# NVIDIA/tensorrt-laboratory

Hardware: NVIDIA H100
Metric: ResNet-50 fp16 b=8 inferences/sec (higher is better)
Workload: dtype f16

## Files before the change

### __graft_entry__.py

```python
from __future__ import annotations

import os
import re
import shutil
import subprocess
import sysconfig
import sys

ROOT = os.path.dirname(os.path.abspath(__file__))
PKG = os.path.join(ROOT, "tensorrt_laboratory_b200")
CSRC = os.path.join(PKG, "csrc")
LIB = os.path.join(PKG, "libb200infer.so")

NVCC_FLAGS = [
    "-gencode", "arch=compute_90a,code=sm_90a", "-lineinfo", "-O3", "-std=c++17",
    "-Xcompiler", "-fPIC,-Wall,-Wno-unused-function", "-cudart", "static",
]


def _nvcc() -> str:
    for cand in (os.environ.get("NVCC"), shutil.which("nvcc"), "/usr/local/cuda/bin/nvcc"):
        if cand and os.path.exists(cand):
            return cand
    raise RuntimeError("nvcc not found")
# ... 20 lines not shown

def _all_deps():
    deps = []
    for root, _, files in os.walk(CSRC):
        deps += [os.path.join(root, f) for f in files if f.endswith((".cu", ".cc", ".h", ".cuh", ".hpp"))]
    deps.append(os.path.join(ROOT, "include", "b200infer.h"))
    inc = os.path.join(ROOT, "include")
    for root, _, files in os.walk(inc):
        deps += [os.path.join(root, f) for f in files]
    return deps


_CONV_KERNEL = re.compile(r"conv|net_f16_tcgen05|attention_f16_wgmma|embed_ln|layernorm_h8|pooler")


def _ptxas_violations(log: str):
    bad = [line.strip() for line in log.splitlines() if "(C7520)" in line]
    func = None
    for line in log.splitlines():
        m = re.search(r"Function properties for (\S+)", line)
        if m:
            func = m.group(1)
            continue
        m = re.search(r"(\d+) bytes spill stores, (\d+) bytes spill loads", line)
        if m and func and _CONV_KERNEL.search(func) and (int(m.group(1)) or int(m.group(2))):
            bad.append(f"{func}: {line.strip()}")
    return bad


def _compile_object(cmd, obj: str, verbose: bool) -> None:
    r = subprocess.run(cmd + ["-Xptxas", "-v"], capture_output=True, text=True)
    log = r.stdout + r.stderr
    shown = [line for line in log.splitlines() if verbose or not (line.startswith("ptxas info") or "bytes stack frame" in line)]
    if shown:
        sys.stderr.write("\n".join(shown) + "\n")
    if r.returncode:
        raise subprocess.CalledProcessError(r.returncode, cmd)
    bad = _ptxas_violations(log)
    if bad:
        os.remove(obj)
        raise RuntimeError(f"{os.path.basename(obj)}: ptxas reports serialised wgmma or spilling convolution / transformer kernels:\n  " +
                           "\n  ".join(bad))


def build(force: bool = False, verbose: bool = False) -> None:
    nvcc = _nvcc()
    objdir = os.path.join(ROOT, "build", "obj")
    os.makedirs(objdir, exist_ok=True)
    deps = _all_deps()
    objs = []
    for src in _sources():
        obj = os.path.join(objdir, os.path.relpath(src, CSRC).replace(os.sep, "_") + ".o")
        objs.append(obj)
        if force or _stale(obj, deps):
            cmd = [nvcc] + NVCC_FLAGS + ["-I", os.path.join(ROOT, "include"), "-I", CSRC]
            if src.endswith(".cc"):
# ... 52 lines not shown
```

### tensorrt_laboratory_b200/csrc/engine.cu

```cuda
#include <cuda.h>
#include <cuda_runtime.h>
#include <stdarg.h>
#include <stdio.h>
#include <stdlib.h>
#include <string.h>

#include <algorithm>
#include <map>
#include <memory>
#include <mutex>
#include <string>
#include <vector>

#include "../../include/b200infer.h"
#include "kernels.h"
#include "plan_format.h"

#include "b2_internal.h"

namespace b2i {
thread_local std::string g_err;
int fail(int code, const char* fmt, ...) {
    char buf[1024];
    va_list ap;
// ... 695 lines not shown
        if (cout_phys % bn || (group_span && group_span % bn)) continue;
        if (honor_forced && c->force_bn && bn != c->force_bn) continue;
        const int tiles = m_tiles * (cout_phys / bn);
        for (int splits = 1; splits <= 8; ++splits) {
            if (honor_forced && c->force_splits && !group_span ? splits != c->force_splits : splits != 1) continue;
            if (splits > 1 && (kb != 64 || kblocks / splits < 4 || tiles * splits > 160 || tiles > kMaxSplitTiles ||
                               size_t(tiles) * splits * 128 * bn * 4 > kSplitWorkspaceBytes))
                continue;
            const int kpc = (kblocks + splits - 1) / splits;
            if (splits > 1 && (splits - 1) * kpc >= kblocks) continue;
            for (int st : stgs) {
                if (!b2k::conv_config_exists(bn, kb, st)) continue;
                if (b2k::conv_smem_bytes(bn, st, residual) > kSmemLimit) continue;
                if (honor_forced && c->force_stages && st != c->force_stages) continue;
                if (!(honor_forced && c->force_stages) && !stage_depth_useful(bn, kb, st, kpc)) continue;
                const double smem = b2k::conv_smem_bytes(bn, st, residual);
                int per_sm = int(double(kSmemLimit) / smem);
                per_sm = std::min(per_sm, bn <= 64 ? 2 : 1);
                per_sm = std::max(1, std::min(per_sm, 8));
                const int ctas = tiles * splits;
                const int waves = (ctas + g_sms * per_sm - 1) / (g_sms * per_sm);
                const int sharing = std::max(1, std::min(per_sm, (ctas + g_sms - 1) / g_sms));
                const double stage_bytes = 16384.0 + bn * 128.0;
                const double t_kb = std::max(stage_bytes / (70000.0 / sharing), 1.0 / st);
                double t_epi = 0.6 + bn / 64.0 * 0.4 + (residual ? 0.4 : 0.0);
                if (splits > 1) t_epi += 1.0 + 0.3 * splits;
                const double t_cta = 2.0 + kpc * t_kb + t_epi;
                double total = waves * t_cta;
                const double traffic = double(ctas) * kpc * stage_bytes;
                total = std::max(total, traffic / 5.0e6 + 2.0);
                if (total < best.est_us) best = ConvConfig{bn, st, splits, total};
            }
        }
    }
// ... 290 lines not shown
        const uint64_t pix = uint64_t(r.cin_phys), rowb = uint64_t(ti.w) * pix, imgb = uint64_t(ti.h) * rowb;
        rc = make_map_im2col(&cl.mapA, tptr(r.in), int(r.cin_phys), int(ti.w), int(ti.h), batch, pix, rowb, imgb, op.kh(), op.kw(), op.sh(),
                             op.sw(), op.ph(), op.pw_lo(), op.pw_hi(), 128, 128, CU_TENSOR_MAP_SWIZZLE_128B, true);
    }
    if (rc) return rc;
    rc = make_map_2d(&cl.mapOut, tptr(r.out), r.cout_phys, uint64_t(M), 128, 128, CU_TENSOR_MAP_SWIZZLE_128B, true);
    if (rc) return rc;
    if (r.res >= 0) rc = make_map_2d(&cl.mapRes, tptr(r.res), r.cout_phys, uint64_t(M), 128, 128, CU_TENSOR_MAP_SWIZZLE_128B, true);
    else cl.mapRes = cl.mapOut;
    return rc;
}

struct TuneTimer {
    const int ns;
    const int iters = std::max(4, env_int("B2_TUNE_ITERS", 12));
    const int reps = std::max(1, env_int("B2_TUNE_REPS", 2));
    std::vector<cudaStream_t> ss;
    std::vector<cudaEvent_t> done;
    cudaEvent_t e0 = nullptr, e1 = nullptr;

    explicit TuneTimer(const b2_context* c) : ns(std::max(1, std::min(c->autotune, 8))), ss(size_t(ns), nullptr), done(size_t(ns), nullptr) {}
    ~TuneTimer() {
        for (auto s : ss)
            if (s) cudaStreamDestroy(s);
        for (auto d : done)
            if (d) cudaEventDestroy(d);
        if (e0) cudaEventDestroy(e0);
        if (e1) cudaEventDestroy(e1);
    }
    int init() {
        bool ok = cudaEventCreate(&e0) == cudaSuccess && cudaEventCreate(&e1) == cudaSuccess;
        for (int i = 0; i < ns && ok; ++i)
            ok = cudaStreamCreateWithFlags(&ss[size_t(i)], cudaStreamNonBlocking) == cudaSuccess &&
                 cudaEventCreateWithFlags(&done[size_t(i)], cudaEventDisableTiming) == cudaSuccess;
        if (ok) return B2_OK;
        cudaGetLastError();
        return fail(B2_ECUDA, "autotune: cannot create streams/events");
    }
    template <class F>
    cudaError_t time(F launch, float* ms) {
        int rc = 0;
        for (int i = 0; i < 2 && !rc; ++i)
            for (int k = 0; k < ns && !rc; ++k) rc = launch(k, ss[size_t(k)]);
        for (auto s : ss) cudaStreamSynchronize(s);
        *ms = 1e30f;
        cudaError_t se = cudaSuccess;
        for (int rep = 0; rep < reps && !rc && se == cudaSuccess; ++rep) {
            cudaEventRecord(e0, ss[0]);
            for (int k = 1; k < ns; ++k) cudaStreamWaitEvent(ss[size_t(k)], e0, 0);
            for (int i = 0; i < iters && !rc; ++i)
                for (int k = 0; k < ns && !rc; ++k) rc = launch(k, ss[size_t(k)]);
            for (int k = 1; k < ns; ++k) {
                cudaEventRecord(done[size_t(k)], ss[size_t(k)]);
                cudaStreamWaitEvent(ss[0], done[size_t(k)], 0);
            }
            cudaEventRecord(e1, ss[0]);
            se = cudaStreamSynchronize(ss[0]);
            float t = 0.f;
            if (se == cudaSuccess && cudaEventElapsedTime(&t, e0, e1) == cudaSuccess) *ms = std::min(*ms, t);
        }
        return rc ? cudaError_t(rc) : se;
    }
    double us_per_launch(double ms) const { return ms * 1e3 / (iters * ns); }
};

int autotune_conv(b2_context* c, const Op& op, int batch, int fixed_splits, ConvConfig* best_out) {
    const b2plan::OpRec& r = op.r;
    const Tensor& to = c->e->tensors[r.out];
    const int M = batch * int(to.h) * int(to.w);
    TuneTimer tt(c);
    int status = tt.init();
    if (status) return status;
    const int verbose = env_int("B2_TUNE_VERBOSE", 0);
    ConvConfig best = *best_out;
    double best_ms = 1e30;
// ... 1377 lines not shown
    const size_t bytes = size_t(run->ctas) * 64 * sizeof(long long);
    B2_CUDA(cudaMalloc(&d, bytes));
    cudaMemset(d, 0, bytes);
    cudaStream_t s = static_cast<cudaStream_t>(stream_);
    run->args.dbg = d;
    int rc = run_all(c, *plan, bindings, s);
    cudaError_t se = cudaStreamSynchronize(s);
    run->args.dbg = nullptr;
    if (!rc && se == cudaSuccess) cudaMemcpy(out, d, bytes, cudaMemcpyDeviceToHost);
    cudaFree(d);
    if (rc) return rc;
    if (se != cudaSuccess) return fail(B2_ECUDA, "debug launch failed: %s", cudaGetErrorString(se));
    return B2_OK;
}

const char* b2_context_launch_name(b2_context* c, int batch, int i) {
    static thread_local std::string s;
    const Launch* L = get_launch(c, batch, i);
    if (!L) return nullptr;
    static const char* kinds[] = {"input_cast", "conv_tcgen05", "conv_simt", "maxpool", "avgpool", "fc", "softmax", "output_cast", "net_tcgen05", "tail_pool_fc_softmax",
                                  "quantize", "conv_i8_tcgen05", "avgpool_i8", "output_cast_i8", "embed_ln", "layernorm", "attention_f16_wgmma",
                                  "pooler", "output_cast_rows"};
    s = std::string(kinds[L->kind]) + ":" + L->name;
    if (L->kind == L_CONV_TC)
        s += " bn=" + std::to_string(L->conv.bn) + " kb=" + std::to_string(L->conv.kb) +
             " st=" + std::to_string(L->conv.stages) + "x" + std::to_string(L->conv.sps) +
             (L->conv.ws_ctas ? " ws=" + std::to_string(L->conv.ws_ctas) : std::string()) +
             (L->conv.cn > 1 ? " cn=" + std::to_string(L->conv.cn) : std::string()) + (L->conv.halo ? " halo" : "") +
             (L->conv.args.a_mode == b2k::A_TILED ? " tiled" : " im2col") +
             " grid=" + std::to_string(L->conv.grid_n) + "x" + std::to_string(L->conv.grid_m) + "x" +
// ... 23 lines not shown
```

### tensorrt_laboratory_b200/csrc/kernels.cu

```cuda
#include "kernels.h"

#include <stdio.h>
#include <stdlib.h>
#include <string.h>

#include "ptx_sm90.cuh"
#include "wgmma_sm90.cuh"

namespace b2k {

template <int BN, int STAGES, int SPS = 1>
struct ConvCfg {
    static constexpr int A_SUBBLK = 128 * 64 * 2;
    static constexpr int B_SUBBLK = BN * 64 * 2;
    static constexpr int A_STAGE = SPS * A_SUBBLK;
    static constexpr int B_STAGE = SPS * B_SUBBLK;
    static constexpr int PIPE_BYTES = STAGES * (A_STAGE + B_STAGE);
    static constexpr int TILE_BYTES = 128 * BN * 2;
    static_assert(TILE_BYTES <= PIPE_BYTES, "the output staging tile reuses the pipeline buffers");
};

__host__ __device__ constexpr int conv_smem_layout_bytes(int bn, int stages, bool residual, int sps = 1) {
    return stages * sps * (128 * 64 * 2 + bn * 64 * 2) + (residual ? 128 * bn * 2 : 0) + 256 + bn * 4 + 1024;
}

constexpr int kConvThreads = 384;
constexpr int kConsumerWarps = 8;

struct FragPos {
    int row0, col0;
    __device__ FragPos(int consumer_warp, int lane)
        : row0(64 * (consumer_warp >> 2) + 16 * (consumer_warp & 3) + (lane >> 2)), col0(2 * (lane & 3)) {}
};

template <int BN, int KB, int STAGES, int SPS, int CN = 1, bool DBG = false, int AV = 0, bool GELU = false>
__global__ void __launch_bounds__(kConvThreads, BN <= 64 ? 2 : 1)
conv_f16_tcgen05(const __grid_constant__ CUtensorMap mapA, const __grid_constant__ CUtensorMap mapB,
                 const __grid_constant__ CUtensorMap mapOut, const __grid_constant__ CUtensorMap mapRes,
                 const ConvArgs p) {
    static_assert(SPS == 1 || KB == 64, "multi-sub-block stages exist for the 64-wide K path only");
    using Cfg = ConvCfg<BN, STAGES, SPS>;
    constexpr int TPS = 64 / KB;
    constexpr int A_SUB = 128 * KB * 2;
    constexpr int B_SUB = BN * KB * 2;
    constexpr int OW = BN >= 64 ? 64 : 32;
    constexpr int OROWB = OW * 2;
    constexpr int NBOX = BN / OW;

    extern __shared__ uint8_t smem_raw[];
    uint8_t* smem = smem_raw + ((1024u - (smem_u32(smem_raw) & 1023u)) & 1023u);
    const bool has_res = p.residual != nullptr;
// ... 42 lines not shown
    if (threadIdx.x == 0) {
        tma_prefetch_desc(&mapA);
        tma_prefetch_desc(&mapB);
        tma_prefetch_desc(&mapOut);
        if (has_res) tma_prefetch_desc(&mapRes);
        for (int s = 0; s < STAGES; ++s) {
            mbar_init(&full_bar[s], 1);
            mbar_init(&empty_bar[s], static_cast<uint32_t>(kConsumerWarps * cn));
        }
        mbar_init(res_bar, 1);
        fence_barrier_init();
        fence_proxy_async();
    }
    __syncthreads();
    if (cn > 1) cluster_sync_all();
    if (warp == 3) {
#pragma unroll
        for (int i = 0; i < BN / 32; ++i) s_bias[lane + 32 * i] = __ldg(p.bias + n0 + lane + 32 * i);
    }
    if (p.pdl_trigger == 0) pdl_launch_dependents();
    if (dbg && threadIdx.x == 0) dbg[1] = clock64();

    auto sub_tiles = [&](int kb) -> int {
        if (KB == 64) return 1;
        const int n = p.taps_phys - kb * TPS;
        return n > TPS ? TPS : n;
    };
    const bool skip_a = DBG && KB == 64 && (p.dbg_mode & 2), skip_b = DBG && KB == 64 && (p.dbg_mode & 4);
    auto stage_bytes = [&](int kb) -> uint32_t {
        if (KB == 64) {
            const int ns = subs_in_step((kb - kb_begin) / SPS);
// ... 13 lines not shown
                } else {
                    tma_load_2d(&mapB, &full_bar[s], b_dst + u * Cfg::B_SUBBLK, (kb + u) * 64, n0);
                }
            }
        } else {
            const int nt = sub_tiles(kb);
            for (int t = 0; t < nt; ++t) tma_load_2d(&mapB, &full_bar[s], b_dst + t * B_SUB, (kb * TPS + t) * KB, n0);
        }
    };
    auto load_residual = [&]() {
        mbar_expect_tx(res_bar, Cfg::TILE_BYTES);
#pragma unroll
        for (int b = 0; b < NBOX; ++b) tma_load_2d(&mapRes, res_bar, sRes + b * (128 * OROWB), n0 + b * OW, m0);
    };

    if (warp == 0) {
        {
            int img0 = 0, p0 = 0, q0 = 0;
            const int slice_rows = 128 / cn;
            int ms = m0 + static_cast<int>(crank) * slice_rows;
            const uint32_t slice_off = crank * static_cast<uint32_t>(slice_rows) * 128u;
            if (!a_tiled) {
                if (ms >= p.M) ms = 0;
                img0 = ms / p.HoWo;
                const int rem = ms - img0 * p.HoWo;
                p0 = rem / p.Wo;
                q0 = rem - p0 * p.Wo;
            }
            const int base_w = q0 * p.stride_w - p.pad_w;
            const int base_h = p0 * p.stride_h - p.pad_h;
            int cur_cb = 0, cur_r = 0, cur_sx = 0;
// ... 73 lines not shown
                    mbar_expect_tx(&full_bar[s], stage_bytes(kb_begin + i * SPS));
                    load_a(kb_begin + i * SPS, s);
                    if (!kSplitProducers) load_b(kb_begin + i * SPS, s);
                }
                __syncwarp();
                if (dbg) {
                    c3 = clock64();
                    tw += c1 - c0, tl += c3 - c1;
                }
            }
            if (dbg && lane == 0) dbg[11] = tw, dbg[12] = te, dbg[13] = tl;
        }
        __syncwarp();
    }

    const int cw = warp - 4;
    float acc[BN / 2];
    if (warp >= 4) {
        const uint32_t wg = static_cast<uint32_t>(cw >> 2);
        auto release_stage = [&](int st) {
            __syncwarp();
            if (lane == 0) {
                if (cn > 1) {
                    for (uint32_t r = 0; r < static_cast<uint32_t>(cn); ++r) mbar_arrive_cluster(&empty_bar[st], r);
                } else {
                    mbar_arrive(&empty_bar[st]);
                }
            }
        };
        long long mw = 0, mi = 0;
        for (int i = 0; i < nk; ++i) {
            const int s = i % STAGES;
            const uint32_t ph = (i / STAGES) & 1;
// ... 34 lines not shown
                wgmma_wait<0>();
                release_stage(0);
            } else {
                wgmma_wait<1>();
                if (i > 0) release_stage((i - 1) % STAGES);
            }
            if (dbg) mi += clock64() - m1c;
        }
        if constexpr (STAGES > 1) {
            wgmma_wait<0>();
            if (nk > 0) release_stage((nk - 1) % STAGES);
        }
        if (dbg && cw == 0 && lane == 0) dbg[4] = clock64(), dbg[14] = mw, dbg[15] = mi;
    }

    if (warp == 3 && KB == 64) {
        for (int i = 0; i < nk; ++i) {
            const int s = i % STAGES;
            if (i >= STAGES) mbar_wait(&empty_bar[s], ((i / STAGES) & 1) ^ 1);
            if (elect_one_sync()) load_b(kb_begin + i * SPS, s);
            __syncwarp();
        }
    }

    pdl_wait();
    __syncthreads();
    if (dbg && threadIdx.x == 128) dbg[5] = clock64();
    if (p.pdl_trigger == 1) pdl_launch_dependents();
    const FragPos fp(cw, lane);

    auto finish_pair = [&](int row, int col, float v0, float v1) {
        const int box = col / OW;
        const int chunk = (col % OW) / 8;
        const uint32_t so = static_cast<uint32_t>(box * (128 * OROWB)) + swz_off<OROWB>(row, chunk) + (col % 8) * 2;
        v0 += s_bias[col];
        v1 += s_bias[col + 1];
        if (has_res) {
            const float2 rf = __half22float2(*reinterpret_cast<const __half2*>(sRes + so));
            v0 += rf.x;
            v1 += rf.y;
        }
        if constexpr (GELU) {
            v0 = gelu_erf(v0);
            v1 = gelu_erf(v1);
        } else if (p.relu) {
            v0 = fmaxf(v0, 0.0f);
            v1 = fmaxf(v1, 0.0f);
        }
        *reinterpret_cast<__half2*>(sOut + so) = __floats2half2_rn(v0, v1);
    };

    bool do_store = true;
    if (!split) {
        if (warp >= 4) {
            if (has_res) mbar_wait(res_bar, 0);
#pragma unroll
            for (int j = 0; j < BN / 8; ++j)
#pragma unroll
                for (int h = 0; h < 2; ++h) finish_pair(fp.row0 + 8 * h, 8 * j + fp.col0, acc[4 * j + 2 * h], acc[4 * j + 2 * h + 1]);
        }
    } else {
        const int tile = blockIdx.y * gridDim.x + blockIdx.x;
        float* ws_tile = p.workspace + static_cast<size_t>(tile) * p.splits * (128 * BN);
        if (warp >= 4) {
            float* mine = ws_tile + static_cast<size_t>(blockIdx.z) * (128 * BN);
#pragma unroll
            for (int j = 0; j < BN / 8; ++j)
#pragma unroll
                for (int h = 0; h < 2; ++h)
                    __stcg(reinterpret_cast<float2*>(mine + (fp.row0 + 8 * h) * BN + 8 * j + fp.col0),
                           make_float2(acc[4 * j + 2 * h], acc[4 * j + 2 * h + 1]));
        }
        __syncthreads();
        if (threadIdx.x == 0) {
            __threadfence();
            const int prev = atomicAdd(p.tile_counters + tile, 1);
            const uint32_t last = (prev == p.splits - 1) ? 1u : 0u;
            if (last) {
                p.tile_counters[tile] = 0;
                if (has_res) load_residual();
            }
            *last_flag = last;
        }
        __syncthreads();
        do_store = *last_flag != 0;
        if (do_store && warp >= 4) {
            __threadfence();
            if (has_res) mbar_wait(res_bar, 0);
#pragma unroll 4
            for (int j = 0; j < BN / 8; ++j) {
#pragma unroll
                for (int h = 0; h < 2; ++h) {
                    const int row = fp.row0 + 8 * h, col = 8 * j + fp.col0;
                    float f0 = 0.f, f1 = 0.f;
                    for (int sp = 0; sp < p.splits; ++sp) {
                        const float2 t = __ldcg(reinterpret_cast<const float2*>(ws_tile + static_cast<size_t>(sp) * (128 * BN) + row * BN + col));
                        f0 += t.x;
                        f1 += t.y;
                    }
                    finish_pair(row, col, f0, f1);
                }
            }
        }
    }
    if (dbg && threadIdx.x == 128) dbg[6] = clock64();
    if (p.pdl_trigger == 2) pdl_launch_dependents();
    fence_proxy_async();
    __syncthreads();
    if (threadIdx.x == 0 && do_store) {
#pragma unroll
        for (int b = 0; b < NBOX; ++b) tma_store_2d(&mapOut, sOut + b * (128 * OROWB), n0 + b * OW, m0);
        tma_store_commit_and_wait_read();
    }
    if (cn > 1) {
        if (warp == 1) {
            const int first = nk > STAGES ? nk - STAGES : 0;
            for (int i = first; i < nk; ++i) mbar_wait(&empty_bar[i % STAGES], (i / STAGES) & 1);
        }
        __syncthreads();
        cluster_sync_all();
    }
    if (dbg && threadIdx.x == 128) {
        dbg[7] = clock64();
        unsigned long long gt;
        asm volatile("mov.u64 %0, %%globaltimer;" : "=l"(gt));
        dbg[9] = static_cast<long long>(gt);
    }
}

__host__ __device__ constexpr int conv_ws_smem_bytes(int bn, int stages, int sps, bool residual) {
    return stages * sps * (128 * 64 * 2 + bn * 64 * 2) + 2 * 128 * bn * 2 + (residual ? 2 * 128 * bn * 2 : 0) + 256 + 1024;
}

template <int BN, int STAGES, int SPS>
__global__ void __launch_bounds__(kConvThreads, 1)
conv_f16_tcgen05_ws(const __grid_constant__ CUtensorMap mapA, const __grid_constant__ CUtensorMap mapOut,
                    const __grid_constant__ CUtensorMap mapRes, const ConvArgs p) {
    constexpr int A_SUBBLK = 128 * 64 * 2;
    constexpr int B_SUBBLK = BN * 64 * 2;
    constexpr int A_STAGE = SPS * A_SUBBLK;
    constexpr int B_STAGE = SPS * B_SUBBLK;
    constexpr int PIPE_BYTES = STAGES * (A_STAGE + B_STAGE);
    constexpr int TILE_BYTES = 128 * BN * 2;
    constexpr int OW = BN >= 64 ? 64 : 32;
    constexpr int OROWB = OW * 2;
    constexpr int NBOX = BN / OW;

    extern __shared__ uint8_t smem_raw[];
    uint8_t* smem = smem_raw + ((1024u - (smem_u32(smem_raw) & 1023u)) & 1023u);
    const bool has_res = p.residual != nullptr;
// ... 207 lines not shown
        if (e0) tma_store_wait_read0();
        if (rec) dbg[2] = clock64(), dbg[3] = d_tiles, dbg[4] = d_mma, dbg[5] = d_res, dbg[6] = d_a, dbg[7] = d_math, dbg[8] = d_b, dbg[10] = w_ops;
    }
    __syncthreads();
}

constexpr int kStemRows = 7;
constexpr int kStemStride = 2;
constexpr int kStemASub = 128 * 32 * 2;
constexpr int kStemBSub = 64 * 32 * 2;
constexpr int kStemTile = 128 * 64 * 2;
__host__ __device__ constexpr int conv_stem_ws_smem_bytes() {
    return kStemWsRing * kStemASub + kStemRows * kStemBSub + 2 * kStemTile + 512 + 1024;
}

__global__ void __launch_bounds__(kConvThreads, 1)
conv_stem_ws_tcgen05(const __grid_constant__ CUtensorMap mapA, const __grid_constant__ CUtensorMap mapB,
                     const __grid_constant__ CUtensorMap mapOut, const ConvArgs p) {
    const int Ho = p.HoWo / p.Wo;
    const int images = p.M / p.HoWo;
    const int band = min(Ho, (images * Ho + static_cast<int>(gridDim.x) - 1) / static_cast<int>(gridDim.x));
    const int bands_per_image = (Ho + band - 1) / band;
    const int num_items = images * bands_per_image;
    if (static_cast<int>(blockIdx.x) >= num_items) return;
    auto item_rows = [&](int item, int& img, int& p0) -> int {
        img = item / bands_per_image;
        p0 = (item - img * bands_per_image) * band;
        return min(band, Ho - p0);
    };

    extern __shared__ uint8_t smem_raw[];
// ... 117 lines not shown
}

constexpr int kHaloMaxCBlocks = 8;
__host__ __device__ constexpr int halo_b_stages(int bn) { return bn >= 256 ? 3 : 4; }
__host__ __device__ constexpr int halo_a_stage_bytes(int w, int r) {
    const int loaded = (r + 2) * (w + 2);
    const int touched = 128 + 2 * (w + 2) + 2;
    const int rows = loaded > touched ? loaded : touched;
    return (rows * 128 + 1023) / 1024 * 1024;
}
__host__ __device__ constexpr int halo_smem_bytes(int bn, int w, int r, int cblocks) {
    return cblocks * halo_a_stage_bytes(w, r) + halo_b_stages(bn) * bn * 128 + 256 + bn * 4 + 1024;
}

template <int BN>
__global__ void __launch_bounds__(kConvThreads, 1)
conv3x3_halo_tcgen05(const __grid_constant__ CUtensorMap mapIn, const __grid_constant__ CUtensorMap mapOut, const ConvArgs p) {
    constexpr int NB = halo_b_stages(BN);
    constexpr int B_BLK = BN * 128;
    constexpr int OW = 64;
    constexpr int NBOX = BN / OW;

    extern __shared__ uint8_t smem_raw[];
    uint8_t* smem = smem_raw + ((1024u - (smem_u32(smem_raw) & 1023u)) & 1023u);
    const int W = p.Wo, Wp = p.Wo + 2, R = p.halo_rows;
    const int a_stage = halo_a_stage_bytes(W, R);
    const int cblocks = p.cblocks;
    uint8_t* sA = smem;
    uint8_t* sB = smem + cblocks * a_stage;
    uint8_t* sOut = smem;
    uint8_t* tail = sB + NB * B_BLK;
// ... 14 lines not shown
    if (threadIdx.x == 0) {
        tma_prefetch_desc(&mapIn);
        tma_prefetch_desc(&mapOut);
        for (int s = 0; s < cblocks; ++s) mbar_init(&a_full[s], 1);
        for (int s = 0; s < NB; ++s) {
            mbar_init(&b_full[s], 1);
            mbar_init(&b_empty[s], kConsumerWarps);
        }
        fence_barrier_init();
        fence_proxy_async();
    }
    __syncthreads();
    if (p.pdl_trigger == 0) pdl_launch_dependents();

    float acc[BN / 2];
    if (warp == 0) {
        const uint32_t halo_bytes = static_cast<uint32_t>((R + 2) * Wp * 128);
        pdl_wait();
        if (elect_one_sync()) {
            for (int cb = 0; cb < cblocks; ++cb) {
                mbar_expect_tx(&a_full[cb], halo_bytes);
                tma_load_4d(&mapIn, &a_full[cb], sA + cb * a_stage, cb * 64, -1, h0 - 1, img);
            }
        }
        __syncwarp();
    } else if (warp >= 4) {
        const uint32_t wg_off = static_cast<uint32_t>((warp - 4) >> 2) * 8192u;
        int i = 0;
#pragma unroll 1
        for (int tap = 0; tap < 9; ++tap) {
            const int r = tap / 3, sx = tap - r * 3;
            const uint32_t tap_off = static_cast<uint32_t>((r * Wp + sx) * 128);
#pragma unroll 1
            for (int cb = 0; cb < cblocks; ++cb, ++i) {
                const int sb = i % NB;
                if (tap == 0) mbar_wait(&a_full[cb], 0);
                mbar_wait(&b_full[sb], (i / NB) & 1);
                const uint32_t a_addr = smem_u32(sA + cb * a_stage) + tap_off + wg_off;
                const uint32_t b_addr = smem_u32(sB + sb * B_BLK);
                wgmma_fence();
#pragma unroll
                for (int j = 0; j < 4; ++j) {
                    const uint64_t ad = make_wgmma_desc(a_addr + j * 32, 16, 1024, WG_SW128);
                    const uint64_t bd = make_wgmma_desc(b_addr + j * 32, 16, 1024, WG_SW128);
                    wgmma_f16<BN>(acc, ad, bd, (i > 0 || j > 0) ? 1u : 0u);
                }
                wgmma_commit();
                wgmma_wait<1>();
                __syncwarp();
                if (i > 0 && lane == 0) mbar_arrive(&b_empty[(i - 1) % NB]);
            }
        }
        wgmma_wait<0>();
        __syncwarp();
        if (lane == 0) mbar_arrive(&b_empty[(nsteps - 1) % NB]);
    } else if (warp == 3) {
        for (int i = lane; i < BN; i += 32) s_bias[i] = __ldg(p.bias + n0 + i);
        for (int i = 0; i < nsteps; ++i) {
            const int sb = i % NB;
            if (i >= NB) mbar_wait(&b_empty[sb], ((i / NB) & 1) ^ 1);
            if (elect_one_sync()) {
                mbar_expect_tx(&b_full[sb], B_BLK);
                bulk_load_1d(&b_full[sb], sB + sb * B_BLK, p.wpacked + (static_cast<size_t>(i) * (p.Cout >> 5) + (n0 >> 5)) * 4096,
                             B_BLK);
            }
            __syncwarp();
        }
    }

    pdl_wait();
    __syncthreads();
    if (p.pdl_trigger == 1) pdl_launch_dependents();
    if (warp >= 4) {
        const FragPos fp(warp - 4, lane);
#pragma unroll
        for (int j = 0; j < BN / 8; ++j) {
#pragma unroll
            for (int h = 0; h < 2; ++h) {
                const int row = fp.row0 + 8 * h, col = 8 * j + fp.col0;
                const uint32_t so = static_cast<uint32_t>((col / OW) * (128 * 128)) + swz_off<128>(row, (col % OW) / 8) + (col % 8) * 2;
                float v0 = acc[4 * j + 2 * h] + s_bias[col], v1 = acc[4 * j + 2 * h + 1] + s_bias[col + 1];
                if (p.relu) {
                    v0 = fmaxf(v0, 0.0f);
                    v1 = fmaxf(v1, 0.0f);
                }
                *reinterpret_cast<__half2*>(sOut + so) = __floats2half2_rn(v0, v1);
            }
        }
    }
    fence_proxy_async();
    __syncthreads();
    if (threadIdx.x == 0) {
#pragma unroll
        for (int b = 0; b < NBOX; ++b) tma_store_4d(&mapOut, sOut + b * (128 * 128), n0 + b * OW, 0, h0, img);
        tma_store_commit_and_wait_read();
    }
}

static bool g_use_pdl = true;
void set_pdl(bool on) { g_use_pdl = on; }
bool get_pdl() { return g_use_pdl; }

template <typename Kern, typename... Args>
static int launch_kernel_cluster(Kern kern, dim3 grid, dim3 block, size_t smem, cudaStream_t stream, bool pdl, unsigned cluster_x,
                                 Args... args) {
    cudaLaunchConfig_t cfg = {};
    cfg.gridDim = grid;
// ... 40 lines not shown
        return launch_kernel_cluster(conv_f16_tcgen05<BN, KB, STAGES, SPS, 1, true>, grid, dim3(kConvThreads), smem, stream, true, 1u, L.mapA,
                                     L.mapB, L.mapOut, L.mapRes, L.args);
    if constexpr (CN == 1 && KB == 64) {
        if (L.args.wpacked != nullptr) {
            if (L.args.a_mode == A_TILED)
                return launch_kernel_cluster(conv_f16_tcgen05<BN, KB, STAGES, SPS, 1, false, 2>, grid, dim3(kConvThreads), smem, stream, true, 1u,
                                             L.mapA, L.mapB, L.mapOut, L.mapRes, L.args);
            return launch_kernel_cluster(conv_f16_tcgen05<BN, KB, STAGES, SPS, 1, false, 1>, grid, dim3(kConvThreads), smem, stream, true, 1u,
                                         L.mapA, L.mapB, L.mapOut, L.mapRes, L.args);
        }
    }
    return launch_kernel_cluster(conv_f16_tcgen05<BN, KB, STAGES, SPS, CN>, grid, dim3(kConvThreads), smem, stream, true,
                                 static_cast<unsigned>(CN), L.mapA, L.mapB, L.mapOut, L.mapRes, L.args);
}

template <int BN, int KB, int STAGES, int SPS, int CN = 1>
static int init_one() {
    const int want = conv_smem_layout_bytes(BN, STAGES, true, SPS);
    const int bytes = want > 227 * 1024 ? conv_smem_layout_bytes(BN, STAGES, false, SPS) : want;
    if (CN == 1) {
        int e = static_cast<int>(cudaFuncSetAttribute(conv_f16_tcgen05<BN, KB, STAGES, SPS, 1, true>,
                                                      cudaFuncAttributeMaxDynamicSharedMemorySize, bytes));
        if (e) return e;
        if constexpr (KB == 64) {
            if ((e = static_cast<int>(cudaFuncSetAttribute(conv_f16_tcgen05<BN, KB, STAGES, SPS, 1, false, 1>,
                                                           cudaFuncAttributeMaxDynamicSharedMemorySize, bytes)))) return e;
            if ((e = static_cast<int>(cudaFuncSetAttribute(conv_f16_tcgen05<BN, KB, STAGES, SPS, 1, false, 2>,
                                                           cudaFuncAttributeMaxDynamicSharedMemorySize, bytes)))) return e;
            if ((e = static_cast<int>(cudaFuncSetAttribute(conv_f16_tcgen05<BN, KB, STAGES, SPS, 1, false, 2, true>,
                                                           cudaFuncAttributeMaxDynamicSharedMemorySize, bytes)))) return e;
        }
    }
    return static_cast<int>(cudaFuncSetAttribute(conv_f16_tcgen05<BN, KB, STAGES, SPS, CN>, cudaFuncAttributeMaxDynamicSharedMemorySize, bytes));
}

int conv_smem_bytes(int bn, int stages, bool residual, int sps) { return conv_smem_layout_bytes(bn, stages, residual, sps); }

#define B2_FOR_EACH_CONV(X) \
    X(32, 64, 1, 1) X(32, 64, 2, 1) X(32, 64, 4, 1) X(32, 64, 8, 1) \
    X(64, 64, 1, 1) X(64, 64, 2, 1) X(64, 64, 4, 1) X(64, 64, 8, 1) \
    X(128, 64, 1, 1) X(128, 64, 2, 1) X(128, 64, 4, 1) X(256, 64, 2, 1) X(256, 64, 4, 1) \
    X(32, 64, 2, 2) X(32, 64, 4, 2) X(64, 64, 2, 2) X(64, 64, 4, 2) X(128, 64, 2, 2) X(256, 64, 2, 2) \
    X(32, 8, 2, 1) X(32, 8, 4, 1) X(64, 8, 2, 1) X(64, 8, 4, 1) X(64, 8, 8, 1) X(128, 8, 4, 1) \
    X(32, 32, 2, 1) X(32, 32, 4, 1) X(64, 32, 1, 1) X(64, 32, 2, 1) X(64, 32, 4, 1) X(128, 32, 2, 1) X(128, 32, 4, 1)

int conv_halo_smem(int bn, int w, int r, int cblocks) { return halo_smem_bytes(bn, w, r, cblocks); }
bool conv_halo_config_exists(int bn) { return bn == 64 || bn == 128 || bn == 256; }
static int init_conv_halo_kernels() {
    int e;
    if ((e = static_cast<int>(cudaFuncSetAttribute(conv3x3_halo_tcgen05<64>, cudaFuncAttributeMaxDynamicSharedMemorySize, 227 * 1024)))) return e;
    if ((e = static_cast<int>(cudaFuncSetAttribute(conv3x3_halo_tcgen05<128>, cudaFuncAttributeMaxDynamicSharedMemorySize, 227 * 1024)))) return e;
    if ((e = static_cast<int>(cudaFuncSetAttribute(conv3x3_halo_tcgen05<256>, cudaFuncAttributeMaxDynamicSharedMemorySize, 227 * 1024)))) return e;
    return 0;
}
static int launch_conv_halo(const ConvLaunch& L, cudaStream_t stream) {
    const int R = L.args.halo_rows;
    const size_t smem = size_t(halo_smem_bytes(L.bn, L.args.Wo, R, L.args.cblocks));
    if (smem > 227 * 1024 || R < 1 || R * (L.args.Wo + 2) > 128 || L.args.cblocks > kHaloMaxCBlocks) return static_cast<int>(cudaErrorInvalidValue);
    dim3 grid(L.grid_n, L.grid_m, 1);
    switch (L.bn) {
        case 64: return launch_kernel(conv3x3_halo_tcgen05<64>, grid, dim3(kConvThreads), smem, stream, true, L.mapA, L.mapOut, L.args);
        case 128: return launch_kernel(conv3x3_halo_tcgen05<128>, grid, dim3(kConvThreads), smem, stream, true, L.mapA, L.mapOut, L.args);
        case 256: return launch_kernel(conv3x3_halo_tcgen05<256>, grid, dim3(kConvThreads), smem, stream, true, L.mapA, L.mapOut, L.args);
    }
    return static_cast<int>(cudaErrorInvalidValue);
}

#define B2_FOR_EACH_CONV_CLUSTER(X) \
    X(32, 4, 1, 2) X(32, 4, 1, 4) X(64, 1, 1, 2) X(64, 2, 1, 2) X(64, 2, 1, 4) X(64, 2, 2, 2) X(64, 4, 2, 2) X(64, 4, 2, 4) \
    X(128, 2, 1, 2) X(128, 2, 1, 4) X(128, 2, 2, 2)

int init_conv_ws_kernels();
int launch_conv_f16_tcgen05_ws(const ConvLaunch& L, cudaStream_t stream);

int conv_stem_ws_smem() { return conv_stem_ws_smem_bytes(); }
static int launch_conv_stem_ws(const ConvLaunch& L, cudaStream_t stream) {
    const ConvArgs& a = L.args;
    if (L.bn != 64 || a.Cout != 64 || a.Wo > 128 || a.taps != kStemRows || a.stride_h != kStemStride || a.residual != nullptr)
        return static_cast<int>(cudaErrorInvalidValue);
    return launch_kernel(conv_stem_ws_tcgen05, dim3(L.ws_ctas), dim3(kConvThreads), size_t(conv_stem_ws_smem_bytes()), stream, true,
                         L.mapA, L.mapB, L.mapOut, L.args);
}

int init_conv_kernels() {
    int e = init_conv_ws_kernels();
    if (e) return e;
    if ((e = static_cast<int>(cudaFuncSetAttribute(conv_stem_ws_tcgen05, cudaFuncAttributeMaxDynamicSharedMemorySize,
                                                   conv_stem_ws_smem_bytes()))))
        return e;
    if ((e = init_conv_halo_kernels())) return e;
#define B2_INIT(BN_, KB_, ST_, SPS_) \
    if ((e = init_one<BN_, KB_, ST_, SPS_>())) return e;
    B2_FOR_EACH_CONV(B2_INIT)
#undef B2_INIT
#define B2_INIT_CL(BN_, ST_, SPS_, CN_) \
// ... 14 lines not shown
        return static_cast<int>(cudaErrorInvalidValue);
    }
#define B2_CASE(BN_, KB_, ST_, SPS_) \
    if (L.bn == BN_ && L.kb == KB_ && L.stages == ST_ && L.sps == SPS_) return launch_one<BN_, KB_, ST_, SPS_>(L, stream);
    B2_FOR_EACH_CONV(B2_CASE)
#undef B2_CASE
    return static_cast<int>(cudaErrorInvalidValue);
}

#define B2_FOR_EACH_CONV_WS(X) \
    X(32, 4, 1) X(64, 2, 1) X(64, 4, 1) X(64, 2, 2) X(64, 4, 2) X(128, 2, 1) X(128, 4, 1) X(128, 2, 2)

template <int BN, int STAGES, int SPS>
static int launch_one_ws(const ConvLaunch& L, cudaStream_t stream) {
    const size_t smem = size_t(conv_ws_smem_bytes(BN, STAGES, SPS, L.args.residual != nullptr));
    return launch_kernel(conv_f16_tcgen05_ws<BN, STAGES, SPS>, dim3(L.ws_ctas), dim3(kConvThreads), smem, stream, true, L.mapA, L.mapOut,
                         L.mapRes, L.args);
}

int init_conv_ws_kernels() {
    int e = 0;
#define B2_INIT_WS(BN_, ST_, SPS_)                                                                                        \
    {                                                                                                                     \
        const int want = conv_ws_smem_bytes(BN_, ST_, SPS_, true);                                                        \
        e = static_cast<int>(cudaFuncSetAttribute(conv_f16_tcgen05_ws<BN_, ST_, SPS_>,                                    \
                                                  cudaFuncAttributeMaxDynamicSharedMemorySize,                            \
                                                  want > 227 * 1024 ? conv_ws_smem_bytes(BN_, ST_, SPS_, false) : want)); \
        if (e) return e;                                                                                                  \
    }
    B2_FOR_EACH_CONV_WS(B2_INIT_WS)
#undef B2_INIT_WS
// ... 20 lines not shown

bool conv_cluster_config_exists(int bn, int stages, int sps, int cn) {
#define B2_HAS_CL(BN_, ST_, SPS_, CN_) \
    if (bn == BN_ && stages == ST_ && sps == SPS_ && cn == CN_) return true;
    B2_FOR_EACH_CONV_CLUSTER(B2_HAS_CL)
#undef B2_HAS_CL
    return false;
}

bool conv_config_exists(int bn, int kb, int stages, int sps) {
#define B2_HAS(BN_, KB_, ST_, SPS_) \
    if (bn == BN_ && kb == KB_ && stages == ST_ && sps == SPS_) return true;
    B2_FOR_EACH_CONV(B2_HAS)
#undef B2_HAS
    return false;
}

static thread_local int B2_LAUNCH_RC = 0;

template <typename T>
struct Acc;
template <>
struct Acc<float> {
    using type = double;
};
template <>
struct Acc<__half> {
    using type = float;
};
__device__ __forceinline__ float to_f(float v) { return v; }
// ... 779 lines not shown
```

### tensorrt_laboratory_b200/csrc/kernels.h

```cpp
#pragma once
#include <cuda.h>
#include <cuda_fp16.h>
#include <cuda_runtime.h>
#include <stdint.h>

namespace b2k {

enum { A_TILED = 0, A_IM2COL = 1 };

struct ConvArgs {
    const float* bias;
    const __half* residual;
    __half* out;
    int M;
    int Cout;
    int num_kblocks;
    int cblocks;
    int taps;
    int taps_phys;
    int kw;
    int HoWo, Wo;
    int stride_h, stride_w;
    int pad_h, pad_w;
    int relu;
// ... 23 lines not shown
    int stages;
    int sps;
    int grid_m, grid_n;
    int cn;
    int halo;
    int ws_ctas;
};

int launch_conv_f16_tcgen05(const ConvLaunch& L, cudaStream_t stream);
int init_conv_kernels();
bool conv_config_exists(int bn, int kb, int stages, int sps = 1);
int conv_smem_bytes(int bn, int stages, bool residual, int sps = 1);
bool conv_cluster_config_exists(int bn, int stages, int sps, int cn);
bool conv_halo_config_exists(int bn);
int conv_halo_smem(int bn, int w, int r, int cblocks);
bool conv_ws_config_exists(int bn, int stages, int sps);
int conv_ws_smem(int bn, int stages, int sps, bool residual);
constexpr int kStemWsRing = 16;
int conv_stem_ws_smem();
void set_pdl(bool on);
bool get_pdl();

constexpr int kNetMaxLayers = 160;

struct NetLayerInfo {
    const uint8_t* wpacked;
    const float* bias;
    __half* out;
    const __half* residual;
    int M, Cout, num_kblocks, cblocks;
// ... 128 lines not shown
```

Measured before the change: 30120.

## Shrink conv CTAs to 320 threads and raise occupancy with register budgets

Removes two idle warps from the main and halo conv kernels by moving the producer roles to warps 8 and 9 after the 8 consumer warps, cutting the block from 384 to 320 threads. Launch bounds now ask for 3 or 2 resident CTAs for small BN tiles, and the build rejects kernels whose register use exceeds that budget. The planner takes CTAs per SM from the CUDA occupancy API instead of a hand-written heuristic, and the autotuner times a captured CUDA graph with an extra rep. The tighter register caps could force spills or trim unrolling, and the new occupancy figures change which tile configurations the planner picks.

```diff
diff --git a/__graft_entry__.py b/__graft_entry__.py
--- a/__graft_entry__.py
+++ b/__graft_entry__.py
@@ -58,8 +58,17 @@
 _CONV_KERNEL = re.compile(r"conv|net_f16_tcgen05|attention_f16_wgmma|embed_ln|layernorm_h8|pooler")
 
 
+_SHARED_SM_KERNEL = re.compile(r"_ZN3b2k(?:16conv_f16_tcgen05|20conv3x3_halo_tcgen05)ILi(\d+)E")
+_SHARED_SM_THREADS = 320
+
+
+def _shared_sm_register_budget(bn: int):
+    ctas = 3 if bn <= 64 else 2 if bn <= 128 else 1
+    return None if ctas == 1 else 65536 // (_SHARED_SM_THREADS * ctas) // 8 * 8
+
+
 def _ptxas_violations(log: str):
-    bad = [line.strip() for line in log.splitlines() if "(C7520)" in line]
+    bad = [line.strip() for line in log.splitlines() if "(C7520)" in line or "(C7518)" in line]
     func = None
     for line in log.splitlines():
         m = re.search(r"Function properties for (\S+)", line)
@@ -69,6 +78,12 @@
         m = re.search(r"(\d+) bytes spill stores, (\d+) bytes spill loads", line)
         if m and func and _CONV_KERNEL.search(func) and (int(m.group(1)) or int(m.group(2))):
             bad.append(f"{func}: {line.strip()}")
+        m = re.search(r"Used (\d+) registers", line)
+        k = _SHARED_SM_KERNEL.match(func) if (m and func) else None
+        if k:
+            budget = _shared_sm_register_budget(int(k.group(1)))
+            if budget is not None and int(m.group(1)) > budget:
+                bad.append(f"{func}: {m.group(1)} registers, more than the {budget} at which its CTAs share an SM")
     return bad
 
 
@@ -83,7 +98,8 @@
     bad = _ptxas_violations(log)
     if bad:
         os.remove(obj)
-        raise RuntimeError(f"{os.path.basename(obj)}: ptxas reports serialised wgmma or spilling convolution / transformer kernels:\n  " +
+        raise RuntimeError(f"{os.path.basename(obj)}: ptxas reports serialised wgmma, spilling convolution / transformer "
+                           "kernels or tile kernels over their register budget:\n  " +
                            "\n  ".join(bad))
 
 
diff --git a/tensorrt_laboratory_b200/csrc/engine.cu b/tensorrt_laboratory_b200/csrc/engine.cu
--- a/tensorrt_laboratory_b200/csrc/engine.cu
+++ b/tensorrt_laboratory_b200/csrc/engine.cu
@@ -733,10 +733,7 @@
                 if (b2k::conv_smem_bytes(bn, st, residual) > kSmemLimit) continue;
                 if (honor_forced && c->force_stages && st != c->force_stages) continue;
                 if (!(honor_forced && c->force_stages) && !stage_depth_useful(bn, kb, st, kpc)) continue;
-                const double smem = b2k::conv_smem_bytes(bn, st, residual);
-                int per_sm = int(double(kSmemLimit) / smem);
-                per_sm = std::min(per_sm, bn <= 64 ? 2 : 1);
-                per_sm = std::max(1, std::min(per_sm, 8));
+                const int per_sm = std::max(1, b2k::conv_residency(bn, kb, st, 1, residual));
                 const int ctas = tiles * splits;
                 const int waves = (ctas + g_sms * per_sm - 1) / (g_sms * per_sm);
                 const int sharing = std::max(1, std::min(per_sm, (ctas + g_sms - 1) / g_sms));
@@ -1057,7 +1054,7 @@
 struct TuneTimer {
     const int ns;
     const int iters = std::max(4, env_int("B2_TUNE_ITERS", 12));
-    const int reps = std::max(1, env_int("B2_TUNE_REPS", 2));
+    const int reps = std::max(1, env_int("B2_TUNE_REPS", 3));
     std::vector<cudaStream_t> ss;
     std::vector<cudaEvent_t> done;
     cudaEvent_t e0 = nullptr, e1 = nullptr;
@@ -1087,21 +1084,34 @@
             for (int k = 0; k < ns && !rc; ++k) rc = launch(k, ss[size_t(k)]);
         for (auto s : ss) cudaStreamSynchronize(s);
         *ms = 1e30f;
-        cudaError_t se = cudaSuccess;
+        if (rc) return cudaError_t(rc);
+        cudaGraph_t g = nullptr;
+        cudaGraphExec_t ge = nullptr;
+        cudaError_t se = cudaStreamBeginCapture(ss[0], cudaStreamCaptureModeThreadLocal);
+        if (se != cudaSuccess) return se;
+        cudaEventRecord(done[0], ss[0]);
+        for (int k = 1; k < ns; ++k) cudaStreamWaitEvent(ss[size_t(k)], done[0], 0);
+        for (int i = 0; i < iters && !rc; ++i)
+            for (int k = 0; k < ns && !rc; ++k) rc = launch(k, ss[size_t(k)]);
+        for (int k = 1; k < ns; ++k) {
+            cudaEventRecord(done[size_t(k)], ss[size_t(k)]);
+            cudaStreamWaitEvent(ss[0], done[size_t(k)], 0);
+        }
+        se = cudaStreamEndCapture(ss[0], &g);
+        if (!rc && se == cudaSuccess) se = cudaGraphInstantiate(&ge, g, 0);
+        if (!rc && se == cudaSuccess) se = cudaGraphLaunch(ge, ss[0]);
+        if (!rc && se == cudaSuccess) se = cudaStreamSynchronize(ss[0]);
         for (int rep = 0; rep < reps && !rc && se == cudaSuccess; ++rep) {
             cudaEventRecord(e0, ss[0]);
-            for (int k = 1; k < ns; ++k) cudaStreamWaitEvent(ss[size_t(k)], e0, 0);
-            for (int i = 0; i < iters && !rc; ++i)
-                for (int k = 0; k < ns && !rc; ++k) rc = launch(k, ss[size_t(k)]);
-            for (int k = 1; k < ns; ++k) {
-                cudaEventRecord(done[size_t(k)], ss[size_t(k)]);
-                cudaStreamWaitEvent(ss[0], done[size_t(k)], 0);
-            }
+            se = cudaGraphLaunch(ge, ss[0]);
             cudaEventRecord(e1, ss[0]);
-            se = cudaStreamSynchronize(ss[0]);
+            if (se == cudaSuccess) se = cudaStreamSynchronize(ss[0]);
             float t = 0.f;
             if (se == cudaSuccess && cudaEventElapsedTime(&t, e0, e1) == cudaSuccess) *ms = std::min(*ms, t);
         }
+        if (ge) cudaGraphExecDestroy(ge);
+        if (g) cudaGraphDestroy(g);
+        if (rc || se != cudaSuccess) cudaGetLastError();
         return rc ? cudaError_t(rc) : se;
     }
     double us_per_launch(double ms) const { return ms * 1e3 / (iters * ns); }
@@ -2509,6 +2519,17 @@
     return B2_OK;
 }
 
+int b2_debug_conv_residency(int bn, int kb, int stages, int sps, int residual, int halo_w, int halo_rows, int cblocks,
+                            int* ctas_per_sm) {
+    if (!ctas_per_sm) return fail(B2_EINVAL, "null output");
+    const int rc = b2k::init_conv_kernels();
+    if (rc) return fail(B2_ECUDA, "kernel attribute setup failed: %s", cudaGetErrorString(cudaError_t(rc)));
+    *ctas_per_sm = b2k::conv_residency(bn, kb, stages, sps, residual != 0, halo_w, halo_rows, cblocks);
+    if (*ctas_per_sm <= 0)
+        return fail(B2_EINVAL, "no residency for bn=%d kb=%d st=%dx%d res=%d halo_w=%d", bn, kb, stages, sps, residual, halo_w);
+    return B2_OK;
+}
+
 const char* b2_context_launch_name(b2_context* c, int batch, int i) {
     static thread_local std::string s;
     const Launch* L = get_launch(c, batch, i);
diff --git a/tensorrt_laboratory_b200/csrc/kernels.cu b/tensorrt_laboratory_b200/csrc/kernels.cu
--- a/tensorrt_laboratory_b200/csrc/kernels.cu
+++ b/tensorrt_laboratory_b200/csrc/kernels.cu
@@ -3,6 +3,10 @@
 #include <stdio.h>
 #include <stdlib.h>
 #include <string.h>
+
+#include <array>
+#include <map>
+#include <mutex>
 
 #include "ptx_sm90.cuh"
 #include "wgmma_sm90.cuh"
@@ -24,8 +28,12 @@
     return stages * sps * (128 * 64 * 2 + bn * 64 * 2) + (residual ? 128 * bn * 2 : 0) + 256 + bn * 4 + 1024;
 }
 
-constexpr int kConvThreads = 384;
+constexpr int kConvThreads = 320;
 constexpr int kConsumerWarps = 8;
+constexpr int kActWarp = 8;
+constexpr int kWgtWarp = 9;
+__host__ __device__ constexpr int conv_min_ctas(int bn) { return bn <= 64 ? 3 : bn <= 128 ? 2 : 1; }
+constexpr int kConvWsThreads = 384;
 
 struct FragPos {
     int row0, col0;
@@ -34,7 +42,7 @@
 };
 
 template <int BN, int KB, int STAGES, int SPS, int CN = 1, bool DBG = false, int AV = 0, bool GELU = false>
-__global__ void __launch_bounds__(kConvThreads, BN <= 64 ? 2 : 1)
+__global__ void __launch_bounds__(kConvThreads, conv_min_ctas(BN))
 conv_f16_tcgen05(const __grid_constant__ CUtensorMap mapA, const __grid_constant__ CUtensorMap mapB,
                  const __grid_constant__ CUtensorMap mapOut, const __grid_constant__ CUtensorMap mapRes,
                  const ConvArgs p) {
@@ -107,7 +115,7 @@
     }
     __syncthreads();
     if (cn > 1) cluster_sync_all();
-    if (warp == 3) {
+    if (warp == kWgtWarp) {
 #pragma unroll
         for (int i = 0; i < BN / 32; ++i) s_bias[lane + 32 * i] = __ldg(p.bias + n0 + lane + 32 * i);
     }
@@ -151,7 +159,7 @@
         for (int b = 0; b < NBOX; ++b) tma_load_2d(&mapRes, res_bar, sRes + b * (128 * OROWB), n0 + b * OW, m0);
     };
 
-    if (warp == 0) {
+    if (warp == kActWarp) {
         {
             int img0 = 0, p0 = 0, q0 = 0;
             const int slice_rows = 128 / cn;
@@ -255,9 +263,10 @@
         __syncwarp();
     }
 
-    const int cw = warp - 4;
+    const int cw = warp;
+    const bool consumer = warp < kConsumerWarps;
     float acc[BN / 2];
-    if (warp >= 4) {
+    if (consumer) {
         const uint32_t wg = static_cast<uint32_t>(cw >> 2);
         auto release_stage = [&](int st) {
             __syncwarp();
@@ -322,7 +331,7 @@
         if (dbg && cw == 0 && lane == 0) dbg[4] = clock64(), dbg[14] = mw, dbg[15] = mi;
     }
 
-    if (warp == 3 && KB == 64) {
+    if (warp == kWgtWarp && KB == 64) {
         for (int i = 0; i < nk; ++i) {
             const int s = i % STAGES;
             if (i >= STAGES) mbar_wait(&empty_bar[s], ((i / STAGES) & 1) ^ 1);
@@ -333,7 +342,7 @@
 
     pdl_wait();
     __syncthreads();
-    if (dbg && threadIdx.x == 128) dbg[5] = clock64();
+    if (dbg && threadIdx.x == 0) dbg[5] = clock64();
     if (p.pdl_trigger == 1) pdl_launch_dependents();
     const FragPos fp(cw, lane);
 
@@ -360,7 +369,7 @@
 
     bool do_store = true;
     if (!split) {
-        if (warp >= 4) {
+        if (consumer) {
             if (has_res) mbar_wait(res_bar, 0);
 #pragma unroll
             for (int j = 0; j < BN / 8; ++j)
@@ -370,7 +379,7 @@
     } else {
         const int tile = blockIdx.y * gridDim.x + blockIdx.x;
         float* ws_tile = p.workspace + static_cast<size_t>(tile) * p.splits * (128 * BN);
-        if (warp >= 4) {
+        if (consumer) {
             float* mine = ws_tile + static_cast<size_t>(blockIdx.z) * (128 * BN);
 #pragma unroll
             for (int j = 0; j < BN / 8; ++j)
@@ -380,7 +389,7 @@
                            make_float2(acc[4 * j + 2 * h], acc[4 * j + 2 * h + 1]));
         }
         __syncthreads();
-        if (threadIdx.x == 0) {
+        if (threadIdx.x == kActWarp * 32) {
             __threadfence();
             const int prev = atomicAdd(p.tile_counters + tile, 1);
             const uint32_t last = (prev == p.splits - 1) ? 1u : 0u;
@@ -392,7 +401,7 @@
         }
         __syncthreads();
         do_store = *last_flag != 0;
-        if (do_store && warp >= 4) {
+        if (do_store && consumer) {
             __threadfence();
             if (has_res) mbar_wait(res_bar, 0);
 #pragma unroll 4
@@ -411,24 +420,24 @@
             }
         }
     }
-    if (dbg && threadIdx.x == 128) dbg[6] = clock64();
+    if (dbg && threadIdx.x == 0) dbg[6] = clock64();
     if (p.pdl_trigger == 2) pdl_launch_dependents();
     fence_proxy_async();
     __syncthreads();
-    if (threadIdx.x == 0 && do_store) {
+    if (threadIdx.x == kActWarp * 32 && do_store) {
 #pragma unroll
         for (int b = 0; b < NBOX; ++b) tma_store_2d(&mapOut, sOut + b * (128 * OROWB), n0 + b * OW, m0);
         tma_store_commit_and_wait_read();
     }
     if (cn > 1) {
-        if (warp == 1) {
+        if (warp == kWgtWarp) {
             const int first = nk > STAGES ? nk - STAGES : 0;
             for (int i = first; i < nk; ++i) mbar_wait(&empty_bar[i % STAGES], (i / STAGES) & 1);
         }
         __syncthreads();
         cluster_sync_all();
     }
-    if (dbg && threadIdx.x == 128) {
+    if (dbg && threadIdx.x == 0) {
         dbg[7] = clock64();
         unsigned long long gt;
         asm volatile("mov.u64 %0, %%globaltimer;" : "=l"(gt));
@@ -441,7 +450,7 @@
 }
 
 template <int BN, int STAGES, int SPS>
-__global__ void __launch_bounds__(kConvThreads, 1)
+__global__ void __launch_bounds__(kConvWsThreads, 1)
 conv_f16_tcgen05_ws(const __grid_constant__ CUtensorMap mapA, const __grid_constant__ CUtensorMap mapOut,
                     const __grid_constant__ CUtensorMap mapRes, const ConvArgs p) {
     constexpr int A_SUBBLK = 128 * 64 * 2;
@@ -679,7 +688,7 @@
     return kStemWsRing * kStemASub + kStemRows * kStemBSub + 2 * kStemTile + 512 + 1024;
 }
 
-__global__ void __launch_bounds__(kConvThreads, 1)
+__global__ void __launch_bounds__(kConvWsThreads, 1)
 conv_stem_ws_tcgen05(const __grid_constant__ CUtensorMap mapA, const __grid_constant__ CUtensorMap mapB,
                      const __grid_constant__ CUtensorMap mapOut, const ConvArgs p) {
     const int Ho = p.HoWo / p.Wo;
@@ -827,7 +836,7 @@
 }
 
 template <int BN>
-__global__ void __launch_bounds__(kConvThreads, 1)
+__global__ void __launch_bounds__(kConvThreads, conv_min_ctas(BN))
 conv3x3_halo_tcgen05(const __grid_constant__ CUtensorMap mapIn, const __grid_constant__ CUtensorMap mapOut, const ConvArgs p) {
     constexpr int NB = halo_b_stages(BN);
     constexpr int B_BLK = BN * 128;
@@ -872,7 +881,7 @@
     if (p.pdl_trigger == 0) pdl_launch_dependents();
 
     float acc[BN / 2];
-    if (warp == 0) {
+    if (warp == kActWarp) {
         const uint32_t halo_bytes = static_cast<uint32_t>((R + 2) * Wp * 128);
         pdl_wait();
         if (elect_one_sync()) {
@@ -882,8 +891,8 @@
             }
         }
         __syncwarp();
-    } else if (warp >= 4) {
-        const uint32_t wg_off = static_cast<uint32_t>((warp - 4) >> 2) * 8192u;
+    } else if (warp < kConsumerWarps) {
+        const uint32_t wg_off = static_cast<uint32_t>(warp >> 2) * 8192u;
         int i = 0;
 #pragma unroll 1
         for (int tap = 0; tap < 9; ++tap) {
@@ -912,7 +921,7 @@
         wgmma_wait<0>();
         __syncwarp();
         if (lane == 0) mbar_arrive(&b_empty[(nsteps - 1) % NB]);
-    } else if (warp == 3) {
+    } else if (warp == kWgtWarp) {
         for (int i = lane; i < BN; i += 32) s_bias[i] = __ldg(p.bias + n0 + i);
         for (int i = 0; i < nsteps; ++i) {
             const int sb = i % NB;
@@ -929,8 +938,8 @@
     pdl_wait();
     __syncthreads();
     if (p.pdl_trigger == 1) pdl_launch_dependents();
-    if (warp >= 4) {
-        const FragPos fp(warp - 4, lane);
+    if (warp < kConsumerWarps) {
+        const FragPos fp(warp, lane);
 #pragma unroll
         for (int j = 0; j < BN / 8; ++j) {
 #pragma unroll
@@ -948,7 +957,7 @@
     }
     fence_proxy_async();
     __syncthreads();
-    if (threadIdx.x == 0) {
+    if (threadIdx.x == kActWarp * 32) {
 #pragma unroll
         for (int b = 0; b < NBOX; ++b) tma_store_4d(&mapOut, sOut + b * (128 * 128), n0 + b * OW, 0, h0, img);
         tma_store_commit_and_wait_read();
@@ -1019,24 +1028,27 @@
                                  static_cast<unsigned>(CN), L.mapA, L.mapB, L.mapOut, L.mapRes, L.args);
 }
 
+template <typename Kern>
+static int set_conv_smem(Kern kern, int bytes) {
+    int e = static_cast<int>(cudaFuncSetAttribute(kern, cudaFuncAttributeMaxDynamicSharedMemorySize, bytes));
+    if (!e) e = static_cast<int>(cudaFuncSetAttribute(kern, cudaFuncAttributePreferredSharedMemoryCarveout, cudaSharedmemCarveoutMaxShared));
+    return e;
+}
+
 template <int BN, int KB, int STAGES, int SPS, int CN = 1>
 static int init_one() {
     const int want = conv_smem_layout_bytes(BN, STAGES, true, SPS);
     const int bytes = want > 227 * 1024 ? conv_smem_layout_bytes(BN, STAGES, false, SPS) : want;
     if (CN == 1) {
-        int e = static_cast<int>(cudaFuncSetAttribute(conv_f16_tcgen05<BN, KB, STAGES, SPS, 1, true>,
-                                                      cudaFuncAttributeMaxDynamicSharedMemorySize, bytes));
+        int e = set_conv_smem(conv_f16_tcgen05<BN, KB, STAGES, SPS, 1, true>, bytes);
         if (e) return e;
         if constexpr (KB == 64) {
-            if ((e = static_cast<int>(cudaFuncSetAttribute(conv_f16_tcgen05<BN, KB, STAGES, SPS, 1, false, 1>,
-                                                           cudaFuncAttributeMaxDynamicSharedMemorySize, bytes)))) return e;
-            if ((e = static_cast<int>(cudaFuncSetAttribute(conv_f16_tcgen05<BN, KB, STAGES, SPS, 1, false, 2>,
-                                                           cudaFuncAttributeMaxDynamicSharedMemorySize, bytes)))) return e;
-            if ((e = static_cast<int>(cudaFuncSetAttribute(conv_f16_tcgen05<BN, KB, STAGES, SPS, 1, false, 2, true>,
-                                                           cudaFuncAttributeMaxDynamicSharedMemorySize, bytes)))) return e;
-        }
-    }
-    return static_cast<int>(cudaFuncSetAttribute(conv_f16_tcgen05<BN, KB, STAGES, SPS, CN>, cudaFuncAttributeMaxDynamicSharedMemorySize, bytes));
+            if ((e = set_conv_smem(conv_f16_tcgen05<BN, KB, STAGES, SPS, 1, false, 1>, bytes))) return e;
+            if ((e = set_conv_smem(conv_f16_tcgen05<BN, KB, STAGES, SPS, 1, false, 2>, bytes))) return e;
+            if ((e = set_conv_smem(conv_f16_tcgen05<BN, KB, STAGES, SPS, 1, false, 2, true>, bytes))) return e;
+        }
+    }
+    return set_conv_smem(conv_f16_tcgen05<BN, KB, STAGES, SPS, CN>, bytes);
 }
 
 int conv_smem_bytes(int bn, int stages, bool residual, int sps) { return conv_smem_layout_bytes(bn, stages, residual, sps); }
@@ -1053,10 +1065,9 @@
 bool conv_halo_config_exists(int bn) { return bn == 64 || bn == 128 || bn == 256; }
 static int init_conv_halo_kernels() {
     int e;
-    if ((e = static_cast<int>(cudaFuncSetAttribute(conv3x3_halo_tcgen05<64>, cudaFuncAttributeMaxDynamicSharedMemorySize, 227 * 1024)))) return e;
-    if ((e = static_cast<int>(cudaFuncSetAttribute(conv3x3_halo_tcgen05<128>, cudaFuncAttributeMaxDynamicSharedMemorySize, 227 * 1024)))) return e;
-    if ((e = static_cast<int>(cudaFuncSetAttribute(conv3x3_halo_tcgen05<256>, cudaFuncAttributeMaxDynamicSharedMemorySize, 227 * 1024)))) return e;
-    return 0;
+    if ((e = set_conv_smem(conv3x3_halo_tcgen05<64>, 227 * 1024))) return e;
+    if ((e = set_conv_smem(conv3x3_halo_tcgen05<128>, 227 * 1024))) return e;
+    return set_conv_smem(conv3x3_halo_tcgen05<256>, 227 * 1024);
 }
 static int launch_conv_halo(const ConvLaunch& L, cudaStream_t stream) {
     const int R = L.args.halo_rows;
@@ -1083,7 +1094,7 @@
     const ConvArgs& a = L.args;
     if (L.bn != 64 || a.Cout != 64 || a.Wo > 128 || a.taps != kStemRows || a.stride_h != kStemStride || a.residual != nullptr)
         return static_cast<int>(cudaErrorInvalidValue);
-    return launch_kernel(conv_stem_ws_tcgen05, dim3(L.ws_ctas), dim3(kConvThreads), size_t(conv_stem_ws_smem_bytes()), stream, true,
+    return launch_kernel(conv_stem_ws_tcgen05, dim3(L.ws_ctas), dim3(kConvWsThreads), size_t(conv_stem_ws_smem_bytes()), stream, true,
                          L.mapA, L.mapB, L.mapOut, L.args);
 }
 
@@ -1128,7 +1139,7 @@
 template <int BN, int STAGES, int SPS>
 static int launch_one_ws(const ConvLaunch& L, cudaStream_t stream) {
     const size_t smem = size_t(conv_ws_smem_bytes(BN, STAGES, SPS, L.args.residual != nullptr));
-    return launch_kernel(conv_f16_tcgen05_ws<BN, STAGES, SPS>, dim3(L.ws_ctas), dim3(kConvThreads), smem, stream, true, L.mapA, L.mapOut,
+    return launch_kernel(conv_f16_tcgen05_ws<BN, STAGES, SPS>, dim3(L.ws_ctas), dim3(kConvWsThreads), smem, stream, true, L.mapA, L.mapOut,
                          L.mapRes, L.args);
 }
 
@@ -1179,6 +1190,42 @@
     B2_FOR_EACH_CONV(B2_HAS)
 #undef B2_HAS
     return false;
+}
+
+int conv_residency(int bn, int kb, int stages, int sps, bool residual, int halo_w, int halo_rows, int cblocks) {
+    static std::mutex mu;
+    static std::map<std::array<int, 8>, int> cache;
+    const std::array<int, 8> key{bn, kb, stages, sps, residual ? 1 : 0, halo_w, halo_rows, cblocks};
+    {
+        std::lock_guard<std::mutex> lock(mu);
+        const auto it = cache.find(key);
+        if (it != cache.end()) return it->second;
+    }
+    const void* fn = nullptr;
+    int smem = 0;
+    if (halo_w > 0) {
+        smem = halo_smem_bytes(bn, halo_w, halo_rows, cblocks);
+        if (bn == 64) fn = reinterpret_cast<const void*>(conv3x3_halo_tcgen05<64>);
+        if (bn == 128) fn = reinterpret_cast<const void*>(conv3x3_halo_tcgen05<128>);
+        if (bn == 256) fn = reinterpret_cast<const void*>(conv3x3_halo_tcgen05<256>);
+    } else {
+        smem = conv_smem_layout_bytes(bn, stages, residual, sps);
+#define B2_FN(BN_, KB_, ST_, SPS_) \
+    if (bn == BN_ && kb == KB_ && stages == ST_ && sps == SPS_) fn = reinterpret_cast<const void*>(conv_f16_tcgen05<BN_, KB_, ST_, SPS_>);
+        B2_FOR_EACH_CONV(B2_FN)
+#undef B2_FN
+    }
+    if (!fn || smem > 227 * 1024) return 0;
+    int n = 0;
+    if (cudaOccupancyMaxActiveBlocksPerMultiprocessor(&n, fn, kConvThreads, static_cast<size_t>(smem)) != cudaSuccess) {
+        cudaGetLastError();
+        return 0;
+    }
+    if (n > 0) {
+        std::lock_guard<std::mutex> lock(mu);
+        cache[key] = n;
+    }
+    return n;
 }
 
 static thread_local int B2_LAUNCH_RC = 0;
diff --git a/tensorrt_laboratory_b200/csrc/kernels.h b/tensorrt_laboratory_b200/csrc/kernels.h
--- a/tensorrt_laboratory_b200/csrc/kernels.h
+++ b/tensorrt_laboratory_b200/csrc/kernels.h
@@ -61,6 +61,7 @@
 bool conv_cluster_config_exists(int bn, int stages, int sps, int cn);
 bool conv_halo_config_exists(int bn);
 int conv_halo_smem(int bn, int w, int r, int cblocks);
+int conv_residency(int bn, int kb, int stages, int sps, bool residual, int halo_w = 0, int halo_rows = 0, int cblocks = 0);
 bool conv_ws_config_exists(int bn, int stages, int sps);
 int conv_ws_smem(int bn, int stages, int sps, bool residual);
 constexpr int kStemWsRing = 16;
```

After: 31830, median of 6. 1.06x the previous value.
